# OpenMined/PIR

Measured on AMD Instinct MI355X. Metric: PIR queries/sec (ms/query in ms_per_step), N=4096 DB=2^20 x 288B d=2, higher is better.
Workload: dtype u64; 1 GPU; N=4096, 2 RNS data primes (36,36 bit | special 37 bit), t=24 bit, DB=2^20 x 288B, d=2, dims=[162, 162], num_pt=26215, 64 queries/step (whole job), 16 in flight per GPU (BASELINE.json configs[2]); workers=16, dist_mode=single, exchange=none, parallelism=single GPU, database_copies_in_hbm=operand layout only (u64 staging released)

## Files before the change

### pir_amd/csrc/scan_mfma.hip

```cpp
#include <hip/hip_runtime.h>

#include <stdlib.h>

#include <algorithm>

#include "arith.h"
#include "kernels.h"

namespace pirgpu {

typedef int v4i __attribute__((ext_vector_type(4)));
typedef unsigned __int128 u128;

#ifndef PIRGPU_SCAN_DIRECT
#define PIRGPU_SCAN_DIRECT 0
#endif
#ifndef PIRGPU_SCAN_PAD
#define PIRGPU_SCAN_PAD 1
#endif

__host__ __device__ __forceinline__ size_t db_tile_offset(uint32_t j, uint32_t rt, uint32_t kg, uint32_t a, uint32_t TB,
                                                          uint32_t RT, uint32_t KG, uint32_t GC) {
  const uint32_t ch = kg / GC, kg0 = ch * GC;
  const uint32_t gc = KG - kg0 < GC ? KG - kg0 : GC;
  return ((size_t)j * RT * KG + (size_t)RT * kg0 + (size_t)rt * gc + (kg - kg0)) * TB + (size_t)a * 256;
}

template <int L>
__host__ __device__ __forceinline__ constexpr int64_t top4_vmax() {
  int64_t p = 1;
  for (int a = 0; a < L - 1; ++a) p *= 256;
  return 7 * p + 127 * ((p - 1) / 255);
}
__host__ __device__ __forceinline__ constexpr uint32_t tile_bytes(uint32_t L, bool top4) {
  return top4 ? (L - 1) * 256 + 128 : L * 256;
}
typedef int v2i __attribute__((ext_vector_type(2)));
__device__ __forceinline__ uint32_t sx4(uint32_t v) {
  return v | (((v >> 3) & 0x01010101u) * 0xF0u);
}
__device__ __forceinline__ v4i expand_top4(v2i w) {
  const uint32_t w0 = (uint32_t)w[0], w1 = (uint32_t)w[1];
  return v4i{(int)sx4(w0 & 0x0F0F0F0Fu), (int)sx4((w0 >> 4) & 0x0F0F0F0Fu), (int)sx4(w1 & 0x0F0F0F0Fu),
              (int)sx4((w1 >> 4) & 0x0F0F0F0Fu)};
}
__device__ __forceinline__ v2i pack_top4(const uint8_t (&o)[16]) {
  uint32_t w[2] = {0, 0};
#pragma unroll
  for (int h = 0; h < 2; ++h)
#pragma unroll
    for (int i = 0; i < 4; ++i)
      w[h] |= (uint32_t)((o[8 * h + i] & 0xF) | ((o[8 * h + 4 + i] & 0xF) << 4)) << (8 * i);
  return v2i{(int)w[0], (int)w[1]};
}

template <int L, bool TOP4 = false>
__device__ __forceinline__ void to_digits(uint64_t x, uint64_t q, int8_t (&d)[L]) {
  int64_t v = TOP4 ? ((int64_t)x > top4_vmax<L>() ? (int64_t)x - (int64_t)q : (int64_t)x)
                   : (x > (q >> 1) ? (int64_t)x - (int64_t)q : (int64_t)x);
#pragma unroll
  for (int a = 0; a < L; ++a) {
    d[a] = (int8_t)(v & 0xFF);
    v = (v - d[a]) >> 8;
  }
}

template <int L, bool TOP4>
__global__ void __launch_bounds__(256)
db_pack_kernel(const DevParams* __restrict__ P, const uint64_t* __restrict__ db, uint8_t* __restrict__ dbp,
               uint32_t rows, uint32_t cols, uint32_t kN, uint32_t RT, uint32_t KG, uint32_t GC, uint32_t slot0) {
  constexpr uint32_t TB = tile_bytes(L, TOP4);
  const uint32_t j = slot0 + blockIdx.x * 16 + (threadIdx.x & 15);
  const uint32_t r16 = threadIdx.x >> 4;
  const uint32_t rt = blockIdx.y, kg = blockIdx.z;
  const uint32_t r = rt * 16 + r16;
  const uint64_t q = P->mod[j >> P->logN].q;
  uint8_t o[L][16];
#pragma unroll
  for (int t = 0; t < 16; ++t) {
    const uint32_t c = kg * 16 + t;
    uint64_t x = 0;
    if (r < rows && c < cols) x = db[((size_t)r * cols + c) * kN + j];
    int8_t d[L];
    to_digits<L, TOP4>(x, q, d);
#pragma unroll
    for (int a = 0; a < L; ++a) o[a][t] = (uint8_t)d[a];
  }
#pragma unroll
  for (int a = 0; a < L; ++a) {
    if (TOP4 && a == L - 1) {
      *reinterpret_cast<v2i*>(dbp + db_tile_offset(j - slot0, rt, kg, a, TB, RT, KG, GC) + r16 * 8) = pack_top4(o[a]);
    } else {
      v4i v;
      __builtin_memcpy(&v, o[a], 16);
      *reinterpret_cast<v4i*>(dbp + db_tile_offset(j - slot0, rt, kg, a, TB, RT, KG, GC) + r16 * 16) = v;
    }
  }
}

template <int L, bool TOP4>
__global__ void __launch_bounds__(256)
sel_pack_kernel(const DevParams* __restrict__ P, MfmaPtrs sv, uint32_t nq, uint8_t* __restrict__ selp, uint32_t cols,
                uint32_t kN, uint32_t KG, int sel_f64, SliceMap map) {
  constexpr uint32_t TB = tile_bytes(L, TOP4);
  const uint32_t j = blockIdx.x * 16 + (threadIdx.x & 15);
  const uint32_t x = threadIdx.x >> 4;
  const uint32_t kg = blockIdx.y;
  const uint64_t q = P->mod[j >> P->logN].q;
  const uint32_t qi = x >> 1, comp = x & 1;
  if (qi >= nq) return;
  const uint64_t* src = (const uint64_t*)sv.p[qi];
  uint8_t o[L][16];
#pragma unroll
  for (int t = 0; t < 16; ++t) {
    const uint32_t c = kg * 16 + t;
    uint64_t v = 0;
    if (c < cols) v = src[((size_t)c * 2 + comp) * kN + j];
    if (sel_f64) v = f64_to_u64(__longlong_as_double((long long)v));
    int8_t d[L];
    to_digits<L, TOP4>(v, q, d);
#pragma unroll
    for (int b = 0; b < L; ++b) o[b][t] = (uint8_t)d[b];
  }
  uint32_t jl = j;
  size_t piece = 0;
  if (map.n) {
    uint32_t r = 0;
    while (r + 1 < map.n && j >= map.cut[r + 1]) ++r;
    jl = j - map.cut[r];
    piece = map.off[r];
  }
  uint8_t* blk = selp + piece + ((size_t)jl * KG + kg) * TB;
#pragma unroll
  for (int b = 0; b < L; ++b) {
    if (TOP4 && b == L - 1) {
      *reinterpret_cast<v2i*>(blk + b * 256 + x * 8) = pack_top4(o[b]);
    } else {
      v4i v;
      __builtin_memcpy(&v, o[b], 16);
      *reinterpret_cast<v4i*>(blk + b * 256 + x * 16) = v;
    }
  }
}

template <int L, bool TOP4>
__global__ void __launch_bounds__(256)
db_unpack_kernel(const DevParams* __restrict__ P, const uint8_t* __restrict__ dbp, uint64_t* __restrict__ out,
                 uint32_t r, uint32_t c, uint32_t kN, uint32_t RT, uint32_t KG, uint32_t GC) {
  constexpr uint32_t TB = tile_bytes(L, TOP4);
  const uint32_t j = blockIdx.x * 256 + threadIdx.x;
  if (j >= kN) return;
  const uint64_t q = P->mod[j >> P->logN].q;
  const uint8_t* blk = dbp + db_tile_offset(j, r >> 4, c >> 4, 0, TB, RT, KG, GC);
  const uint8_t* p = blk + (r & 15) * 16 + (c & 15);
  int64_t v = 0;
#pragma unroll
  for (int a = L - 1; a >= 0; --a) {
    if (TOP4 && a == L - 1) {
      const uint32_t cc = c & 15;
      const uint8_t byte = blk[(size_t)a * 256 + (r & 15) * 8 + (cc >> 3) * 4 + (cc & 3)];
      const int nib = (cc & 4) ? (byte >> 4) : (byte & 0xF);
      v = nib >= 8 ? nib - 16 : nib;
    } else {
      v = v * 256 + (int8_t)p[(size_t)a * 256];
    }
  }
  out[j] = v < 0 ? (uint64_t)(v + (int64_t)q) : (uint64_t)v;
}

__device__ __forceinline__ int row_byte(const uint32_t (&w)[4], int c) { return (int8_t)(w[c >> 2] >> (8 * (c & 3))); }
__device__ __forceinline__ int row_nibble(const uint32_t (&w)[2], int c) {
  const int nib = (int)(w[c >> 3] >> (8 * (c & 3) + ((c & 4) ? 4 : 0))) & 0xF;
  return nib >= 8 ? nib - 16 : nib;
}

template <int L, bool TOP4>
__global__ void __launch_bounds__(256)
db_gather_kernel(const DevParams* __restrict__ P, const uint8_t* __restrict__ dbp, const DbUnit* __restrict__ units,
                 uint64_t* __restrict__ out, uint32_t N, uint32_t RT, uint32_t KG, uint32_t GC) {
  constexpr uint32_t TB = tile_bytes(L, TOP4);
  constexpr int LF = TOP4 ? L - 1 : L;
  const uint32_t j = blockIdx.x * 256 + threadIdx.x;
  if (j >= N) return;
  const DbUnit u = units[blockIdx.y];
  const uint64_t q = P->mod[0].q;
  const uint8_t* blk = dbp + db_tile_offset(j, u.r >> 4, u.kg, 0, TB, RT, KG, GC);
  const uint32_t r16 = u.r & 15;
  uint32_t w[LF][4];
#pragma unroll
  for (int a = 0; a < LF; ++a) {
    const v4i v = *reinterpret_cast<const v4i*>(blk + (size_t)a * 256 + r16 * 16);
#pragma unroll
    for (int x = 0; x < 4; ++x) w[a][x] = (uint32_t)v[x];
  }
  uint32_t w4[2] = {0, 0};
  if constexpr (TOP4) {
    const v2i v = *reinterpret_cast<const v2i*>(blk + (size_t)(L - 1) * 256 + r16 * 8);
    w4[0] = (uint32_t)v[0];
    w4[1] = (uint32_t)v[1];
  }
  uint32_t rank = 0;
#pragma unroll
  for (int cc = 0; cc < 16; ++cc) {
    if (!((u.mask >> cc) & 1)) continue;
    int64_t v = TOP4 ? row_nibble(w4, cc) : row_byte(w[L - 1], cc);
#pragma unroll
    for (int a = L - 2; a >= 0; --a) v = v * 256 + row_byte(w[a], cc);
    out[(size_t)(u.out0 + rank) * N + j] = v < 0 ? (uint64_t)(v + (int64_t)q) : (uint64_t)v;
    ++rank;
  }
}

template <int L, bool TOP4>
__global__ void __launch_bounds__(256)
db_pack_update_kernel(const DevParams* __restrict__ P, const uint64_t* __restrict__ enc, const DbUnit* __restrict__ units,
                      uint8_t* __restrict__ dbp, uint32_t kN, uint32_t slot0, uint32_t nslots, uint32_t RT, uint32_t KG,
                      uint32_t GC) {
  constexpr uint32_t TB = tile_bytes(L, TOP4);
  constexpr int LF = TOP4 ? L - 1 : L;
  const uint32_t jl = blockIdx.x * 256 + threadIdx.x;
  if (jl >= nslots) return;
  const uint32_t j = slot0 + jl;
  const DbUnit u = units[blockIdx.y];
  const uint64_t q = P->mod[j >> P->logN].q;
  uint8_t* blk = dbp + db_tile_offset(jl, u.r >> 4, u.kg, 0, TB, RT, KG, GC);
  const uint32_t r16 = u.r & 15;
  uint32_t w[LF][4];
#pragma unroll
  for (int a = 0; a < LF; ++a) {
    const v4i v = *reinterpret_cast<const v4i*>(blk + (size_t)a * 256 + r16 * 16);
#pragma unroll
    for (int x = 0; x < 4; ++x) w[a][x] = (uint32_t)v[x];
  }
  uint32_t w4[2] = {0, 0};
  if constexpr (TOP4) {
    const v2i v = *reinterpret_cast<const v2i*>(blk + (size_t)(L - 1) * 256 + r16 * 8);
    w4[0] = (uint32_t)v[0];
    w4[1] = (uint32_t)v[1];
  }
  uint32_t rank = 0;
#pragma unroll
  for (int cc = 0; cc < 16; ++cc) {
    if (!((u.mask >> cc) & 1)) continue;
    int8_t d[L];
    to_digits<L, TOP4>(enc[(size_t)(u.out0 + rank) * kN + j], q, d);
    ++rank;
    const uint32_t sh = 8 * (cc & 3);
#pragma unroll
    for (int a = 0; a < LF; ++a) w[a][cc >> 2] = (w[a][cc >> 2] & ~(0xFFu << sh)) | ((uint32_t)(uint8_t)d[a] << sh);
    if constexpr (TOP4) {
      const uint32_t ns = sh + ((cc & 4) ? 4 : 0);
      w4[cc >> 3] = (w4[cc >> 3] & ~(0xFu << ns)) | (((uint32_t)d[L - 1] & 0xFu) << ns);
    }
  }
#pragma unroll
  for (int a = 0; a < LF; ++a)
    *reinterpret_cast<v4i*>(blk + (size_t)a * 256 + r16 * 16) = v4i{(int)w[a][0], (int)w[a][1], (int)w[a][2], (int)w[a][3]};
  if constexpr (TOP4)
    *reinterpret_cast<v2i*>(blk + (size_t)(L - 1) * 256 + r16 * 8) = v2i{(int)w4[0], (int)w4[1]};
}

__device__ __forceinline__ v4i load_tile(const uint8_t* p) {
  return __builtin_nontemporal_load(reinterpret_cast<const v4i*>(p));
}
__device__ __forceinline__ v2i load_tile8(const uint8_t* p) {
  return __builtin_nontemporal_load(reinterpret_cast<const v2i*>(p));
}

struct ChunkPlan {
  uint32_t first[kMaxScanChunks + 1];
  uint32_t nchunks;
};

template <int L, int KS, int NW, bool TOP4, bool F64F = false>
__global__ void __launch_bounds__(NW * 64)
scan_mfma_kernel(const DevParams* __restrict__ P, const uint8_t* __restrict__ dbp, ScanGroups grp, uint32_t rows,
                 uint32_t RT, uint32_t KG, uint64_t chunk_stride, ChunkPlan plan, uint32_t GC, uint32_t slot0,
                 uint32_t nslots, uint64_t out_qstride, uint32_t out_rstride, uint32_t blk_major) {
  constexpr uint32_t TB = tile_bytes(L, TOP4);
  constexpr int LF = TOP4 ? L - 1 : L;
  constexpr int NS = 2 * L - 1;
  constexpr int NG = (NS + 4) / 5;
  constexpr bool kDirect = PIRGPU_SCAN_DIRECT != 0;
  __shared__ __attribute__((aligned(16))) uint64_t stage[kDirect ? 1 : 2][kDirect ? 1 : 16][kDirect ? 1 : 16][NW + PIRGPU_SCAN_PAD];
  const int w = threadIdx.x >> 6, l = threadIdx.x & 63;
  const int g = l >> 4, i16 = l & 15;
  constexpr int LOGNW = NW == 8 ? 3 : 2;
  const uint32_t nblocks = nslots >> LOGNW;
  const uint32_t nunits = nblocks * grp.n;
  uint32_t ch = 0;
  while (ch + 1 < plan.nchunks && blockIdx.x >= plan.first[ch + 1]) ++ch;
  const uint32_t wg_in_chunk = blockIdx.x - plan.first[ch], wgs_in_chunk = plan.first[ch + 1] - plan.first[ch];
  const uint32_t kg0 = ch * GC;
  const uint32_t gc = KG - kg0 < GC ? KG - kg0 : GC;
  const size_t slab = (size_t)RT * KG * TB;
  const size_t chunk_base = (size_t)RT * kg0 * TB;
  const size_t rt_stride = (size_t)gc * TB;
  const uint32_t lane16 = i16 * 16, lane8 = i16 * 8;

  v4i B[KS][L], A[KS][LF];
  v2i A4[KS];
  auto load_B = [&](uint32_t gi, uint32_t jl) {
    const uint8_t* selp = grp.sel[gi];
    const uint32_t nx = 2u * grp.nq[gi];
#pragma unroll
    for (int ks = 0; ks < KS; ++ks) {
      const uint32_t gl = ks * 4 + g, kg = kg0 + gl;
      const uint8_t* blk = selp + ((size_t)jl * KG + kg) * TB;
#pragma unroll
      for (int b = 0; b < L; ++b) {
        B[ks][b] = v4i{0, 0, 0, 0};
        if (gl < gc && (uint32_t)i16 < nx) {
          if (TOP4 && b == L - 1) B[ks][b] = expand_top4(*reinterpret_cast<const v2i*>(blk + b * 256 + lane8));
          else B[ks][b] = *reinterpret_cast<const v4i*>(blk + b * 256 + lane16);
        }
      }
    }
  };
  auto load_A = [&](int ks, const uint8_t* base, uint32_t gl) {
    const uint8_t* blk = base + (size_t)gl * TB;
#pragma unroll
    for (int a = 0; a < LF; ++a) A[ks][a] = load_tile(blk + a * 256 + lane16);
    if constexpr (TOP4) A4[ks] = load_tile8(blk + (L - 1) * 256 + lane8);
  };

#define PIRGPU_UNIT_OF(uu, gi_, blk_)                                  \
  const uint32_t gi_ = blk_major ? (uu) % grp.n : (uu) / nblocks;      \
  const uint32_t blk_ = blk_major ? (uu) / grp.n : (uu) - gi_ * nblocks;
  uint32_t u = wg_in_chunk;
  if (u >= nunits) return;
  {
    PIRGPU_UNIT_OF(u, gi, blk)
    load_B(gi, blk * NW + w);
    const uint8_t* abase = dbp + (size_t)(blk * NW + w) * slab + chunk_base;
#pragma unroll
    for (int ks = 0; ks < KS; ++ks) {
      const uint32_t gl = ks * 4 + g;
#pragma unroll
      for (int a = 0; a < LF; ++a) A[ks][a] = v4i{0, 0, 0, 0};
      A4[ks] = v2i{0, 0};
      if (gl < gc) load_A(ks, abase, gl);
    }
  }

  uint32_t parity = 0;
  for (; u < nunits; u += wgs_in_chunk) {
    PIRGPU_UNIT_OF(u, gi, blk)
    const uint32_t j0 = blk * NW;
    const uint32_t j = slot0 + j0 + w;
    const uint32_t mi = j >> P->logN;
    const ModConst m = P->mod[mi];
    const uint32_t nx = 2u * grp.nq[gi];
    uint64_t* const obase = grp.out[gi] + ch * chunk_stride;
    const uint64_t bias = m.q << (58 - (64 - __builtin_clzll(m.q)));
    [[maybe_unused]] const F64Mod fm{P->tab[mi].qd, P->tab[mi].qinvd};
    [[maybe_unused]] const double fw0 = P->fold_w[mi][0], fw1 = P->fold_w[mi][1], fw2 = P->fold_w[mi][2];
    const uint8_t* abase = dbp + (size_t)(j0 + w) * slab + chunk_base;
    const uint32_t nu = u + wgs_in_chunk;
    const bool has_next = nu < nunits;
    PIRGPU_UNIT_OF(nu, ngi, nblk)
    const uint8_t* nbase = dbp + (size_t)(nblk * NW + w) * slab + chunk_base;

    for (uint32_t rt = 0; rt < RT; ++rt) {
      v4i T[NS];
#pragma unroll
      for (int s = 0; s < NS; ++s) T[s] = v4i{0, 0, 0, 0};
      const bool last = rt + 1 == RT;
      const uint8_t* next_tile = last ? nbase : abase + (size_t)(rt + 1) * rt_stride;
      const bool refill = !last || has_next;
#pragma unroll
      for (int ks = 0; ks < KS; ++ks) {
        [[maybe_unused]] v4i Atop;
        if constexpr (TOP4) Atop = expand_top4(A4[ks]);
#pragma unroll
        for (int off = 0; off < L; ++off)
#pragma unroll
          for (int a = 0; a < L; ++a) {
            const int b = (a + off) % L;
            if (TOP4 && a == L - 1)
              T[a + b] = __builtin_amdgcn_mfma_i32_16x16x64_i8(Atop, B[ks][b], T[a + b], 0, 0, 0);
            else
              T[a + b] = __builtin_amdgcn_mfma_i32_16x16x64_i8(A[ks][a < LF ? a : 0], B[ks][b], T[a + b], 0, 0, 0);
          }
        const uint32_t gl = ks * 4 + g;
        if (refill && gl < gc) load_A(ks, next_tile, gl);
      }
      if (last && has_next) load_B(ngi, nblk * NW + w);
      const int buf = parity;
      parity ^= 1;
#pragma unroll
      for (int i = 0; i < 4; ++i) {
        uint64_t r = 0;
        if constexpr (F64F) {
          constexpr int NC = (NS + 3) / 4;
          double acc = 0.0;
#pragma unroll
          for (int c = NC - 1; c >= 0; --c) {
            double C = 0.0;
#pragma unroll
            for (int s = (4 * c + 3 < NS ? 4 * c + 3 : NS - 1); s >= 4 * c; --s) C = __builtin_fma(C, 256.0, (double)T[s][i]);
            if (c == 0) acc += f64_norm(C, fm);
            else acc += f64_mulmod(C, c == 1 ? fw0 : (c == 2 ? fw1 : fw2), fm);
          }
          r = f64_to_u64(f64_canon(f64_norm(acc, fm), fm));
        } else {
#pragma unroll
          for (int gq = NG - 1; gq >= 0; --gq) {
            int64_t G = 0;
#pragma unroll
            for (int s = gq * 5; s < gq * 5 + 5 && s < NS; ++s) G += (int64_t)T[s][i] << (8 * (s - gq * 5));
            if (gq == NG - 1 && NG > 1) {
              r = (uint64_t)(G + (int64_t)bias);
            } else {
              const u128 v = ((u128)r << 40) + (uint64_t)(G + (int64_t)bias);
              r = reduce128((uint64_t)v, (uint64_t)(v >> 64), m);
            }
          }
        }
        if constexpr (kDirect) {
          const uint32_t row = rt * 16 + g * 4 + i;
          if ((uint32_t)i16 < nx && row < rows)
            obase[(size_t)(i16 >> 1) * out_qstride + ((size_t)row * 2 + (i16 & 1)) * out_rstride + j0 + w] = r;
        } else {
          stage[buf][g * 4 + i][i16][w] = r;
        }
      }
      if constexpr (kDirect) continue;
      __syncthreads();
#pragma unroll
      for (int round = 0; round < 2; ++round) {
        const int run = round * 128 + (threadIdx.x >> (LOGNW - 1));
        const int part = threadIdx.x & (NW / 2 - 1);
        const int r16 = run >> 4, x = run & 15;
        const uint32_t r = rt * 16 + r16;
        if (x < (int)nx && r < rows) {
          typedef unsigned long long u64x2 __attribute__((ext_vector_type(2)));
#if PIRGPU_SCAN_PAD == 2
          const u64x2 v = *reinterpret_cast<const u64x2*>(&stage[buf][r16][x][part * 2]);
#else
          const u64x2 v = {stage[buf][r16][x][part * 2], stage[buf][r16][x][part * 2 + 1]};
#endif
          uint64_t* dst = obase + (size_t)(x >> 1) * out_qstride + ((size_t)r * 2 + (x & 1)) * out_rstride + j0 + part * 2;
          *reinterpret_cast<u64x2*>(dst) = v;
        }
      }
    }
  }
}

#undef PIRGPU_UNIT_OF

__global__ void __launch_bounds__(256)
slots_assemble_kernel(const uint64_t* __restrict__ src, uint64_t* __restrict__ dst, SliceMap map, uint32_t RC, uint32_t kN,
                      uint64_t dst_qstride, uint32_t nq_total, uint32_t q0) {
  const uint32_t j = (blockIdx.x * 256 + threadIdx.x) * 2;
  const uint32_t rc = blockIdx.y, q = blockIdx.z;
  if (j >= kN) return;
  uint32_t h = 0;
  while (h + 1 < map.n && j >= map.cut[h + 1]) ++h;
  const uint32_t c0 = map.cut[h], width = map.cut[h + 1] - c0;
  typedef unsigned long long u64x2 __attribute__((ext_vector_type(2)));
  const uint64_t* s = src + (size_t)nq_total * RC * c0 + ((size_t)(q0 + q) * RC + rc) * width + (j - c0);
  *reinterpret_cast<u64x2*>(dst + (size_t)q * dst_qstride + (size_t)rc * kN + j) =
      __builtin_nontemporal_load(reinterpret_cast<const u64x2*>(s));
}


MfmaGeom mfma_geometry(const DevParams& hp, uint32_t rows, uint32_t cols, int wide_override, bool allow_top4) {
  MfmaGeom gm{};
  uint32_t bits = 0;
  for (uint32_t i = 0; i < hp.k; ++i) bits = std::max<uint32_t>(bits, 64 - (uint32_t)__builtin_clzll(hp.mod[i].q));
  if (bits <= 39) gm.L = 5;
  else if (bits <= 47) gm.L = 6;
  else if (bits <= 55) gm.L = 7;
  else return gm;
  if (rows < 1 || cols < 1) { gm.L = 0; return gm; }
  gm.RT = (rows + 15) / 16;
  gm.KG = (cols + 15) / 16;
  const uint32_t steps = (gm.KG + 3) / 4;
  const uint32_t narrow_ks = gm.L <= 6 ? 3 : 2, wide_ks = gm.L <= 6 ? 7 : 6;
  bool wide = steps > narrow_ks;
  if (wide_override >= 0) wide = wide_override != 0;
  gm.NW = wide ? 4 : 8;
  const uint32_t max_ks = wide ? wide_ks : narrow_ks;
  gm.KS = std::min(max_ks, steps);
  gm.nchunks = (steps + gm.KS - 1) / gm.KS;
  if (gm.nchunks > (uint32_t)kMaxScanChunks) { gm.L = 0; return gm; }
  gm.GC = (gm.KG + gm.nchunks - 1) / gm.nchunks;
  gm.KS = (gm.GC + 3) / 4;
  if (wide && gm.KS < 3) gm.NW = 8;
  gm.top4 = allow_top4 && gm.L <= 6 && bits <= 8 * (gm.L - 1) + 4 ? 1 : 0;
  gm.tile_bytes = tile_bytes(gm.L, gm.top4 != 0);
  const size_t kN = (size_t)hp.k * hp.N;
  gm.db_bytes = kN * gm.RT * gm.KG * gm.tile_bytes;
  gm.sel_bytes = kN * gm.KG * gm.tile_bytes;
  return gm;
}

hipError_t launch_db_pack(hipStream_t st, const DevParams* P, const MfmaGeom& gm, const uint64_t* db, uint8_t* dbp,
                          uint32_t rows, uint32_t cols, uint32_t kN, uint32_t slot0, uint32_t nslots) {
  if (nslots == 0) nslots = kN - slot0;
  if (slot0 % 16 || nslots % 16 || slot0 + nslots > kN) return hipErrorInvalidValue;
  const dim3 grid(nslots / 16, gm.RT, gm.KG);
#define PIRGPU_DBPACK(L_, T_) \
  hipLaunchKernelGGL((db_pack_kernel<L_, T_>), grid, dim3(256), 0, st, P, db, dbp, rows, cols, kN, gm.RT, gm.KG, gm.GC, slot0)
  switch (gm.L) {
    case 5:
      if (gm.top4) PIRGPU_DBPACK(5, true);
      else PIRGPU_DBPACK(5, false);
      break;
    case 6:
      if (gm.top4) PIRGPU_DBPACK(6, true);
      else PIRGPU_DBPACK(6, false);
      break;
    case 7: PIRGPU_DBPACK(7, false); break;
    default: return hipErrorInvalidValue;
  }
#undef PIRGPU_DBPACK
  return hipGetLastError();
}

hipError_t launch_db_unpack(hipStream_t st, const DevParams* P, const MfmaGeom& gm, const uint8_t* dbp, uint64_t* out,
                            uint32_t row, uint32_t col, uint32_t kN) {
  const dim3 grid((kN + 255) / 256);
  switch (gm.L) {
    case 5:
      if (gm.top4) hipLaunchKernelGGL((db_unpack_kernel<5, true>), grid, dim3(256), 0, st, P, dbp, out, row, col, kN, gm.RT, gm.KG, gm.GC);
      else hipLaunchKernelGGL((db_unpack_kernel<5, false>), grid, dim3(256), 0, st, P, dbp, out, row, col, kN, gm.RT, gm.KG, gm.GC);
      break;
    case 6:
      if (gm.top4) hipLaunchKernelGGL((db_unpack_kernel<6, true>), grid, dim3(256), 0, st, P, dbp, out, row, col, kN, gm.RT, gm.KG, gm.GC);
      else hipLaunchKernelGGL((db_unpack_kernel<6, false>), grid, dim3(256), 0, st, P, dbp, out, row, col, kN, gm.RT, gm.KG, gm.GC);
      break;
    case 7: hipLaunchKernelGGL((db_unpack_kernel<7, false>), grid, dim3(256), 0, st, P, dbp, out, row, col, kN, gm.RT, gm.KG, gm.GC); break;
    default: return hipErrorInvalidValue;
  }
  return hipGetLastError();
}

hipError_t launch_db_gather(hipStream_t st, const DevParams* P, const MfmaGeom& gm, const uint8_t* dbp,
                            const DbUnit* units, uint32_t n_units, uint64_t* out, uint32_t N) {
  if (!n_units) return hipSuccess;
  if (n_units > 65535) return hipErrorInvalidValue;
  const dim3 grid((N + 255) / 256, n_units);
#define PIRGPU_DBGATHER(L_, T_) \
  hipLaunchKernelGGL((db_gather_kernel<L_, T_>), grid, dim3(256), 0, st, P, dbp, units, out, N, gm.RT, gm.KG, gm.GC)
  switch (gm.L) {
    case 5:
      if (gm.top4) PIRGPU_DBGATHER(5, true);
      else PIRGPU_DBGATHER(5, false);
      break;
    case 6:
      if (gm.top4) PIRGPU_DBGATHER(6, true);
      else PIRGPU_DBGATHER(6, false);
      break;
    case 7: PIRGPU_DBGATHER(7, false); break;
    default: return hipErrorInvalidValue;
  }
#undef PIRGPU_DBGATHER
  return hipGetLastError();
}

hipError_t launch_db_pack_update(hipStream_t st, const DevParams* P, const MfmaGeom& gm, const uint64_t* enc,
                                 const DbUnit* units, uint32_t n_units, uint8_t* dbp, uint32_t kN, uint32_t slot0,
                                 uint32_t nslots) {
  if (!n_units) return hipSuccess;
  if (nslots == 0) nslots = kN - slot0;
  if (n_units > 65535 || slot0 % 16 || nslots % 16 || slot0 + nslots > kN) return hipErrorInvalidValue;
  const dim3 grid((nslots + 255) / 256, n_units);
#define PIRGPU_DBPACKUPD(L_, T_)                                                                                    \
  hipLaunchKernelGGL((db_pack_update_kernel<L_, T_>), grid, dim3(256), 0, st, P, enc, units, dbp, kN, slot0, nslots, \
                     gm.RT, gm.KG, gm.GC)
  switch (gm.L) {
    case 5:
      if (gm.top4) PIRGPU_DBPACKUPD(5, true);
      else PIRGPU_DBPACKUPD(5, false);
      break;
    case 6:
      if (gm.top4) PIRGPU_DBPACKUPD(6, true);
      else PIRGPU_DBPACKUPD(6, false);
      break;
    case 7: PIRGPU_DBPACKUPD(7, false); break;
    default: return hipErrorInvalidValue;
  }
#undef PIRGPU_DBPACKUPD
  return hipGetLastError();
}

hipError_t launch_sel_pack(hipStream_t st, const DevParams* P, const MfmaGeom& gm, const MfmaPtrs& sv, uint32_t nq,
                           uint8_t* selp, uint32_t cols, uint32_t kN, bool sel_f64, const SliceMap* map) {
  const int f = sel_f64 ? 1 : 0;
  const dim3 grid(kN / 16, gm.KG);
  SliceMap m{};
  if (map) {
    m = *map;
    if (m.n > (uint32_t)kMaxSlices || m.cut[0] != 0 || m.cut[m.n] != kN) return hipErrorInvalidValue;
    for (uint32_t r = 0; r <= m.n; ++r)
      if (m.cut[r] % 16) return hipErrorInvalidValue;
  }
#define PIRGPU_SELPACK(L_, T_) \
  hipLaunchKernelGGL((sel_pack_kernel<L_, T_>), grid, dim3(256), 0, st, P, sv, nq, selp, cols, kN, gm.KG, f, m)
  switch (gm.L) {
    case 5:
      if (gm.top4) PIRGPU_SELPACK(5, true);
      else PIRGPU_SELPACK(5, false);
      break;
    case 6:
      if (gm.top4) PIRGPU_SELPACK(6, true);
      else PIRGPU_SELPACK(6, false);
      break;
    case 7: PIRGPU_SELPACK(7, false); break;
    default: return hipErrorInvalidValue;
  }
#undef PIRGPU_SELPACK
  return hipGetLastError();
}

hipError_t launch_slots_assemble(hipStream_t st, const uint64_t* src, uint64_t* dst, const SliceMap& map, uint32_t RC,
                                 uint32_t kN, uint32_t nq, uint64_t dst_qstride, uint32_t nq_total, uint32_t q0) {
  if (map.n == 0 || map.n > (uint32_t)kMaxSlices || map.cut[0] != 0 || map.cut[map.n] != kN || q0 + nq > nq_total)
    return hipErrorInvalidValue;
  hipLaunchKernelGGL(slots_assemble_kernel, dim3((kN / 2 + 255) / 256, RC, nq), dim3(256), 0, st, src, dst, map, RC, kN,
                     dst_qstride, nq_total, q0);
  return hipGetLastError();
}

static uint32_t scan_wgs_all() {
  static const uint32_t wgs_all = [] {
    const char* v = pirgpu_env("PIRGPU_SCAN_MFMA_WGS");
    if (v && *v) return (uint32_t)strtoul(v, nullptr, 10);
    hipDeviceProp_t prop;
    int dev = 0;
    if (hipGetDevice(&dev) != hipSuccess || hipGetDeviceProperties(&prop, dev) != hipSuccess) return 256u;
    return (uint32_t)prop.multiProcessorCount;
  }();
  return wgs_all;
}

template <int L, int KS, int NW, bool TOP4, bool F64F>
static void launch_scan_mfma_variant(hipStream_t st, const DevParams* P, const MfmaGeom& gm, const uint8_t* dbp,
                                     const ScanGroups& grp, uint32_t rows, uint64_t chunk_stride, uint32_t wgs_req,
                                     uint32_t slot0, uint32_t nslots, uint64_t out_qstride, uint32_t out_rstride,
                                     bool blk_major) {
  const uint32_t wgs = wgs_req ? std::min(wgs_req, scan_wgs_all()) : scan_wgs_all();
  ChunkPlan plan{};
  plan.nchunks = gm.nchunks;
  const uint32_t units = nslots / NW * std::max<uint32_t>(grp.n, 1);
  const uint32_t share = std::min<uint32_t>(units, std::max<uint32_t>(1, wgs / std::min<uint32_t>(gm.nchunks, wgs)));
  for (uint32_t c = 0; c <= gm.nchunks; ++c) plan.first[c] = c * share;
  hipLaunchKernelGGL((scan_mfma_kernel<L, KS, NW, TOP4, F64F>), dim3(gm.nchunks * share), dim3(NW * 64), 0, st, P, dbp, grp,
                     rows, gm.RT, gm.KG, chunk_stride, plan, gm.GC, slot0, nslots, out_qstride, out_rstride,
                     blk_major ? 1u : 0u);
}

hipError_t launch_scan_mfma_groups(hipStream_t st, const DevParams* P, const MfmaGeom& gm, const uint8_t* dbp,
                                   const ScanGroups& grp, uint32_t rows, uint64_t chunk_stride, uint32_t wgs, bool f64_fold,
                                   uint32_t slot0, uint32_t nslots, uint64_t out_qstride, uint32_t out_rstride, bool blk_major) {
  if (grp.n == 0 || grp.n > (uint32_t)kMaxScanGroups || nslots == 0 || nslots % gm.NW) return hipErrorInvalidValue;
#define PIRGPU_MFMA_ARGS st, P, gm, dbp, grp, rows, chunk_stride, wgs, slot0, nslots, out_qstride, out_rstride, blk_major
#define PIRGPU_MFMA_CASE(L_, KS_, NW_)                                                                    \
  if (gm.L == L_ && gm.KS == KS_ && gm.NW == NW_) {                                                                 \
    if constexpr (L_ <= 6) {                                                                                         \
      if (gm.top4) {                                                                                                 \
        if (f64_fold) launch_scan_mfma_variant<L_, KS_, NW_, true, true>(PIRGPU_MFMA_ARGS);                          \
        else launch_scan_mfma_variant<L_, KS_, NW_, true, false>(PIRGPU_MFMA_ARGS);                                  \
        return hipGetLastError();                                                                                    \
      }                                                                                                              \
    }                                                                                                                \
    if (gm.top4) return hipErrorInvalidValue;                                                                        \
    if (f64_fold) launch_scan_mfma_variant<L_, KS_, NW_, false, true>(PIRGPU_MFMA_ARGS);                             \
    else launch_scan_mfma_variant<L_, KS_, NW_, false, false>(PIRGPU_MFMA_ARGS);                                     \
    return hipGetLastError();                                                                                        \
  }
  PIRGPU_MFMA_CASE(5, 1, 8) PIRGPU_MFMA_CASE(5, 2, 8) PIRGPU_MFMA_CASE(5, 3, 8)
  PIRGPU_MFMA_CASE(6, 1, 8) PIRGPU_MFMA_CASE(6, 2, 8) PIRGPU_MFMA_CASE(6, 3, 8)
  PIRGPU_MFMA_CASE(7, 1, 8) PIRGPU_MFMA_CASE(7, 2, 8)
  PIRGPU_MFMA_CASE(5, 3, 4) PIRGPU_MFMA_CASE(5, 4, 4) PIRGPU_MFMA_CASE(5, 5, 4) PIRGPU_MFMA_CASE(5, 6, 4) PIRGPU_MFMA_CASE(5, 7, 4)
  PIRGPU_MFMA_CASE(6, 3, 4) PIRGPU_MFMA_CASE(6, 4, 4) PIRGPU_MFMA_CASE(6, 5, 4) PIRGPU_MFMA_CASE(6, 6, 4) PIRGPU_MFMA_CASE(6, 7, 4)
  PIRGPU_MFMA_CASE(7, 3, 4) PIRGPU_MFMA_CASE(7, 4, 4) PIRGPU_MFMA_CASE(7, 5, 4) PIRGPU_MFMA_CASE(7, 6, 4)
#undef PIRGPU_MFMA_CASE
#undef PIRGPU_MFMA_ARGS
  return hipErrorInvalidValue;
}

hipError_t launch_scan_mfma(hipStream_t st, const DevParams* P, const MfmaGeom& gm, const uint8_t* dbp,
                            const uint8_t* selp, uint64_t* out, uint64_t out_qstride, uint32_t nq, uint32_t rows,
                            uint32_t kN, uint64_t chunk_stride, uint32_t wgs, bool f64_fold) {
  ScanGroups grp{};
  grp.n = 1;
  grp.sel[0] = selp;
  grp.out[0] = out;
  grp.nq[0] = (uint8_t)nq;
  return launch_scan_mfma_groups(st, P, gm, dbp, grp, rows, chunk_stride, wgs, f64_fold, 0, kN, out_qstride, kN, false);
}

}
```

Before: 5482 queries/s.

## Make scan-kernel A-tile refill branchless and specialize the last row tile

Out-of-range k-group lanes are clamped to the last valid group (glc), so A-tile loads always run without per-lane predicates or zero fills. The row-tile loop body becomes a lambda, and the final row tile is instantiated separately with a compile-time flag. Scheduling barriers are placed around the loads and the wave index is made scalar with readfirstlane. The change also reads grp.nq as aligned words, re-reads the WGS environment variable on each call, and adds geometry validation. Clamped lanes now load redundant data, which assumes the matching B entries are zero so the result is unaffected. The sched barriers may also limit the compiler's ability to interleave instructions.

```diff
diff --git a/pir_amd/csrc/scan_mfma.hip b/pir_amd/csrc/scan_mfma.hip
--- a/pir_amd/csrc/scan_mfma.hip
+++ b/pir_amd/csrc/scan_mfma.hip
@@ -267,6 +267,11 @@
   return __builtin_nontemporal_load(reinterpret_cast<const v2i*>(p));
 }
 
+template <bool V>
+struct BoolConst {
+  static constexpr bool value = V;
+};
+
 struct ChunkPlan {
   uint32_t first[kMaxScanChunks + 1];
   uint32_t nchunks;
@@ -283,7 +288,7 @@
   constexpr int NG = (NS + 4) / 5;
   constexpr bool kDirect = PIRGPU_SCAN_DIRECT != 0;
   __shared__ __attribute__((aligned(16))) uint64_t stage[kDirect ? 1 : 2][kDirect ? 1 : 16][kDirect ? 1 : 16][NW + PIRGPU_SCAN_PAD];
-  const int w = threadIdx.x >> 6, l = threadIdx.x & 63;
+  const int w = __builtin_amdgcn_readfirstlane((int)(threadIdx.x >> 6)), l = threadIdx.x & 63;
   const int g = l >> 4, i16 = l & 15;
   constexpr int LOGNW = NW == 8 ? 3 : 2;
   const uint32_t nblocks = nslots >> LOGNW;
@@ -297,12 +302,21 @@
   const size_t chunk_base = (size_t)RT * kg0 * TB;
   const size_t rt_stride = (size_t)gc * TB;
   const uint32_t lane16 = i16 * 16, lane8 = i16 * 8;
-
+  uint32_t glc[KS];
+#pragma unroll
+  for (int ks = 0; ks < KS; ++ks) glc[ks] = (uint32_t)(ks * 4 + g) < gc ? (uint32_t)(ks * 4 + g) : gc - 1;
+
+  static_assert(kMaxScanGroups % 4 == 0 && offsetof(ScanGroups, nq) % 4 == 0, "grp.nq is read by aligned words");
+  auto queries_of = [&](uint32_t gi) -> uint32_t {
+    uint32_t word;
+    __builtin_memcpy(&word, grp.nq + (gi & ~3u), 4);
+    return (word >> (8 * (gi & 3u))) & 0xFFu;
+  };
   v4i B[KS][L], A[KS][LF];
   v2i A4[KS];
   auto load_B = [&](uint32_t gi, uint32_t jl) {
     const uint8_t* selp = grp.sel[gi];
-    const uint32_t nx = 2u * grp.nq[gi];
+    const uint32_t nx = 2u * queries_of(gi);
 #pragma unroll
     for (int ks = 0; ks < KS; ++ks) {
       const uint32_t gl = ks * 4 + g, kg = kg0 + gl;
@@ -335,12 +349,10 @@
     const uint8_t* abase = dbp + (size_t)(blk * NW + w) * slab + chunk_base;
 #pragma unroll
     for (int ks = 0; ks < KS; ++ks) {
-      const uint32_t gl = ks * 4 + g;
-#pragma unroll
-      for (int a = 0; a < LF; ++a) A[ks][a] = v4i{0, 0, 0, 0};
-      A4[ks] = v2i{0, 0};
-      if (gl < gc) load_A(ks, abase, gl);
+      __builtin_amdgcn_sched_barrier(0);
+      load_A(ks, abase, glc[ks]);
     }
+    __builtin_amdgcn_sched_barrier(0);
   }
 
   uint32_t parity = 0;
@@ -350,7 +362,7 @@
     const uint32_t j = slot0 + j0 + w;
     const uint32_t mi = j >> P->logN;
     const ModConst m = P->mod[mi];
-    const uint32_t nx = 2u * grp.nq[gi];
+    const uint32_t nx = 2u * queries_of(gi);
     uint64_t* const obase = grp.out[gi] + ch * chunk_stride;
     const uint64_t bias = m.q << (58 - (64 - __builtin_clzll(m.q)));
     [[maybe_unused]] const F64Mod fm{P->tab[mi].qd, P->tab[mi].qinvd};
@@ -361,13 +373,14 @@
     PIRGPU_UNIT_OF(nu, ngi, nblk)
     const uint8_t* nbase = dbp + (size_t)(nblk * NW + w) * slab + chunk_base;
 
-    for (uint32_t rt = 0; rt < RT; ++rt) {
+    __builtin_amdgcn_s_waitcnt(0x0F70);
+    auto row_tile = [&](const uint32_t rt, auto last_c) {
+      constexpr bool last = decltype(last_c)::value;
       v4i T[NS];
 #pragma unroll
       for (int s = 0; s < NS; ++s) T[s] = v4i{0, 0, 0, 0};
-      const bool last = rt + 1 == RT;
-      const uint8_t* next_tile = last ? nbase : abase + (size_t)(rt + 1) * rt_stride;
-      const bool refill = !last || has_next;
+      const uint8_t* next_tile = abase + (size_t)(last ? rt : rt + 1) * rt_stride;
+      if (last && has_next) next_tile = nbase;
 #pragma unroll
       for (int ks = 0; ks < KS; ++ks) {
         [[maybe_unused]] v4i Atop;
@@ -382,8 +395,8 @@
             else
               T[a + b] = __builtin_amdgcn_mfma_i32_16x16x64_i8(A[ks][a < LF ? a : 0], B[ks][b], T[a + b], 0, 0, 0);
           }
-        const uint32_t gl = ks * 4 + g;
-        if (refill && gl < gc) load_A(ks, next_tile, gl);
+        load_A(ks, next_tile, glc[ks]);
+        __builtin_amdgcn_sched_barrier(0);
       }
       if (last && has_next) load_B(ngi, nblk * NW + w);
       const int buf = parity;
@@ -425,7 +438,7 @@
           stage[buf][g * 4 + i][i16][w] = r;
         }
       }
-      if constexpr (kDirect) continue;
+      if constexpr (kDirect) return;
       __syncthreads();
 #pragma unroll
       for (int round = 0; round < 2; ++round) {
@@ -444,7 +457,9 @@
           *reinterpret_cast<u64x2*>(dst) = v;
         }
       }
-    }
+    };
+    for (uint32_t rt = 0; rt + 1 < RT; ++rt) row_tile(rt, BoolConst<false>{});
+    row_tile(RT - 1, BoolConst<true>{});
   }
 }
 
@@ -626,15 +641,15 @@
 }
 
 static uint32_t scan_wgs_all() {
-  static const uint32_t wgs_all = [] {
-    const char* v = pirgpu_env("PIRGPU_SCAN_MFMA_WGS");
-    if (v && *v) return (uint32_t)strtoul(v, nullptr, 10);
+  if (const char* v = pirgpu_env("PIRGPU_SCAN_MFMA_WGS"))
+    if (*v) return std::max<uint32_t>(1, (uint32_t)strtoul(v, nullptr, 10));
+  static const uint32_t cus = [] {
     hipDeviceProp_t prop;
     int dev = 0;
     if (hipGetDevice(&dev) != hipSuccess || hipGetDeviceProperties(&prop, dev) != hipSuccess) return 256u;
     return (uint32_t)prop.multiProcessorCount;
   }();
-  return wgs_all;
+  return cus;
 }
 
 template <int L, int KS, int NW, bool TOP4, bool F64F>
@@ -657,6 +672,7 @@
                                    const ScanGroups& grp, uint32_t rows, uint64_t chunk_stride, uint32_t wgs, bool f64_fold,
                                    uint32_t slot0, uint32_t nslots, uint64_t out_qstride, uint32_t out_rstride, bool blk_major) {
   if (grp.n == 0 || grp.n > (uint32_t)kMaxScanGroups || nslots == 0 || nslots % gm.NW) return hipErrorInvalidValue;
+  if (gm.nchunks == 0 || gm.GC == 0 || (size_t)(gm.nchunks - 1) * gm.GC >= gm.KG) return hipErrorInvalidValue;
 #define PIRGPU_MFMA_ARGS st, P, gm, dbp, grp, rows, chunk_stride, wgs, slot0, nslots, out_qstride, out_rstride, blk_major
 #define PIRGPU_MFMA_CASE(L_, KS_, NW_)                                                                    \
   if (gm.L == L_ && gm.KS == KS_ && gm.NW == NW_) {                                                                 \
```

New measurement: 5482 queries/s (median of 2 runs). No clear change (+0.0%).
